# jameshball/kidney-diffusion

Measured on AMD Instinct MI355X. Metric: denoising-steps/sec (64->256 SR UNet, bs16), higher is better.
Workload: dtype f32

## Files before the change

### include/kd_engine.h

```cpp
#ifndef KD_ENGINE_H
#define KD_ENGINE_H

#include <stddef.h>
#include <stdint.h>

#ifdef __cplusplus
extern "C" {
#endif

#define KD_MAX_LEVELS 8

const char* kd_last_error(void);
#define KD_ENGINE_ABI_VERSION 2
int kd_version(void);
const char* kd_build_id(void);

typedef struct kd_unet_config {
  int dim;
  int num_levels;
  int dim_mults[KD_MAX_LEVELS];
  int num_resnet_blocks[KD_MAX_LEVELS];
  int layer_attns[KD_MAX_LEVELS];
  int layer_cross_attns[KD_MAX_LEVELS];
  int cond_dim;
// ... 184 lines not shown
                           float* d_part, int B, int H, int W, int heads, void* stream);
int kd_linattn_context(const float* d_k, const float* d_v, int ld, const float* d_part, int HW, const float* d_ck,
                       const float* d_cv, int ldc, int m, const float* d_null_k, const float* d_null_v, float* d_ctx, int B,
                       int heads, void* stream);
int kd_linattn_apply(const float* d_q, int ldq, const float* d_ctx, float* d_out, int ldo, int B, int N, int heads,
                     float scale, int silu, void* stream);
int kd_gn_fold_seg(const double* d_seg0, int nseg0, int nchunk0, float scale0, float ab_mul0, const double* d_seg1, int nseg1,
                   int nchunk1, float scale1, float ab_mul1, const float* d_gamma, const float* d_beta,
                   const float* d_scale_shift, int ld_ss, float* d_ab, float* d_stats, int B, int HW, int C, int G, float eps,
                   void* stream);
float kd_wf_ab_scale(void);
int kd_gn_conv3x3_winograd4_nhwc(const float* d_x, int ldx, const float* d_stats, const float* d_gamma, const float* d_beta,
                                 const float* d_scale_shift, int ld_ss, int skip_c0, float skip_scale, const float* d_w_oihw,
                                 const float* d_bias, const float* d_res, int ldres, float* d_y, double* d_out_seg, int B,
                                 int H, int W, int Cin, int Cout, int G, int gemm_mode, int images_per_set, void* stream);

int kd_init_conv_nchw(const float* d_x, const float* d_w3, const float* d_w7, const float* d_w15,
                      const float* d_bias, float* d_y, int B, int S, int n3, int n7, int n15, void* stream);
int kd_init_conv_planes_nchw(const float* d_x, const float* d_self_cond, const float* d_w3, const float* d_w7,
                             const float* d_w15, int Itot, int c0, const float* d_bias, const float* d_res, float* d_y, int B,
                             int S, int n3, int n7, int n15, int iters, float* ms, void* stream);
int kd_groupnorm_silu_nhwc(const float* d_x, const float* d_gamma, const float* d_beta,
                           const float* d_scale_shift, float* d_y, int B, int HW, int C, int G,
                           float eps, void* stream);
int kd_layernorm(const float* d_x, const float* d_g, const float* d_beta, float* d_y,
                 int rows, int C, float eps, void* stream);
int kd_layernorm_ex(const float* d_x, const float* d_g, const float* d_beta, const float* d_res, float* d_y, int rows, int C,
                    float eps, int in_act, const float* d_g2, float* d_y2, void* stream);
int kd_layernorm_linear_bf16x3(const float* d_x, const float* d_g, const float* d_beta, int rows, int C, float eps, int in_act,
                               const float* d_w, const float* d_bias, const float* d_res, int ldres, float* d_y, int ldy,
// ... 17 lines not shown
```

### kidney-diffusion_amd/csrc/api.inc

```
extern "C" {

const char* kd_last_error(void) { return kd::g_err.c_str(); }
int kd_version(void) { return KD_ENGINE_ABI_VERSION; }

int kd_unet_create(const kd_unet_config_t* cfg, const kd_param_t* params, int n_params, kd_unet_t** out) {
  return kd_unet_create_shared(cfg, params, n_params, nullptr, out);
}

int kd_unet_create_shared(const kd_unet_config_t* cfg, const kd_param_t* params, int n_params,
                          const kd_unet_t* share_with, kd_unet_t** out) {
  return kd_unet_create_self_cond(cfg, params, n_params, share_with, 0, out);
}

int kd_unet_create_self_cond(const kd_unet_config_t* cfg, const kd_param_t* params, int n_params,
                             const kd_unet_t* share_with, int self_cond, kd_unet_t** out) {
  kd_unet_ext_t ext;
  memset(&ext, 0, sizeof ext);
  ext.self_cond = self_cond;
  return kd_unet_create_ext(cfg, params, n_params, share_with, &ext, out);
}

int kd_unet_create_ext(const kd_unet_config_t* cfg, const kd_param_t* params, int n_params, const kd_unet_t* share_with,
                       const kd_unet_ext_t* ext, kd_unet_t** out) {
  const int self_cond = ext ? ext->self_cond : 0;
  if (!cfg || !params || !out) {
    set_error("kd_unet_create: null argument");
    return 1;
  }
  int ndev = 0;
  if (hipGetDeviceCount(&ndev) != hipSuccess || ndev == 0) {
    set_error("kd_unet_create: no HIP device visible — the engine has no CPU path");
    return 1;
  }
  if (share_with && (share_with->self_cond != 0) != (self_cond != 0)) {
    set_error("kd_unet_create: a shared plan must have the same self_cond");
    return 1;
  }
  kd_unet* u = new kd_unet();
  u->cfg = *cfg;
  u->self_cond = self_cond != 0;
  if (ext)
    for (int l = 0; l < KD_MAX_LEVELS; ++l) {
      u->lin_attn[l] = l < cfg->num_levels && ext->use_linear_attn[l] != 0;
      u->lin_cross[l] = l < cfg->num_levels && ext->use_linear_cross_attn[l] != 0;
    }
  u->wstore = share_with ? share_with->wstore : std::make_shared<WeightStore>();
  try {
    Builder b(u);
    for (int i = 0; i < n_params; ++i) {
      if (!params[i].name || !params[i].d_data) throw std::runtime_error("parameter table has a null entry");
      b.params[params[i].name] = {params[i].d_data, params[i].numel};
    }
    b.build();
    u->ws_bytes = b.arena.peak;
// ... 563 lines not shown
                 16 * (nseg0 + (d_seg1 ? nseg1 : 0)) == C,
             "kd_gn_fold_seg: the sources' 16-channel segments must tile the C channels");
  KD_REQUIRE(!d_ab || (d_gamma && d_beta), "kd_gn_fold_seg: the affine needs gamma and beta");
  KD_REQUIRE(!d_scale_shift || ld_ss >= 2 * C, "kd_gn_fold_seg: FiLM rows [scale | shift] need ld_ss >= 2 C");
  SegSrc s0{d_seg0, nseg0, nchunk0, 0, scale0, ab_mul0};
  SegSrc s1{d_seg1, d_seg1 ? nseg1 : 0, d_seg1 ? nchunk1 : 0, 16 * nseg0, scale1, ab_mul1};
  return entry_finish(launch_gn_fold_seg(s0, s1, d_gamma, d_beta, d_scale_shift, ld_ss, d_ab, d_stats, B, C, G,
                                         (double)HW * (C / G), eps, s),
                      s);
}

int kd_gn_conv3x3_winograd4_nhwc(const float* d_x, int ldx, const float* d_stats, const float* d_gamma, const float* d_beta,
                                 const float* d_scale_shift, int ld_ss, int skip_c0, float skip_scale, const float* d_w_oihw,
                                 const float* d_bias, const float* d_res, int ldres, float* d_y, double* d_out_seg, int B,
                                 int H, int W, int Cin, int Cout, int G, int gemm_mode, int images_per_set, void* stream) {
  hipStream_t s = (hipStream_t)stream;
  if (ldx <= 0) ldx = Cin;
  if (ldres <= 0) ldres = Cout;
  const int Bx = images_per_set > 0 ? images_per_set : B;
  KD_REQUIRE(d_x && d_stats && d_gamma && d_beta && d_w_oihw && d_bias && d_y, "kd_gn_conv3x3_winograd4_nhwc: null argument");
  KD_REQUIRE(B > 0 && Bx > 0 && B % Bx == 0, "kd_gn_conv3x3_winograd4_nhwc: images_per_set must divide B");
  KD_REQUIRE(H > 0 && W > 0 && H % 4 == 0 && W % 4 == 0, "Winograd F(4x4,3x3) path needs H % 4 == 0 and W % 4 == 0");
  const int64_t Mt = (int64_t)Bx * (H / 4) * (W / 4);
  KD_REQUIRE(Mt % 128 == 0 && Cin % 32 == 0 && Cout % 64 == 0 && 36 * Mt < 0x7fffffff &&
                 (int64_t)36 * Cout * Cin * 4 < 0x7fffffff,
             "Winograd F(4x4,3x3) path needs images_per_set*H*W/16 % 128 == 0, Cin % 32 == 0, Cout % 64 == 0");
  KD_REQUIRE(gemm_mode == -1 || gemm_mode == 1 || gemm_mode == 2, "kd_gn_conv3x3_winograd4_nhwc: gemm_mode -1, 1 or 2");
  KD_REQUIRE(gemm_mode < 0 || gemm_bf16x3_ok(36, Mt, Cout, Cin),
             "bf16x3 position GEMMs need images_per_set*H*W/16 % 256 == 0, Cout % 128 == 0, Cin % 32 == 0");
  KD_REQUIRE(G > 0 && Cin % G == 0, "kd_gn_conv3x3_winograd4_nhwc: Cin % G == 0");
// ... 4 lines not shown
  KD_REQUIRE(!d_res || (ldres >= Cout && ldres % 2 == 0), "kd_gn_conv3x3_winograd4_nhwc: residual row stride >= Cout, even");
  KD_REQUIRE((((uintptr_t)d_y | (uintptr_t)d_res | (uintptr_t)d_bias) & 7) == 0,
             "kd_gn_conv3x3_winograd4_nhwc: 8-byte aligned y, residual and bias");
  const bool planes = gemm_mode == 1, x3 = gemm_mode > 0;
  EntryBufs bufs;
  float *U = nullptr, *D = nullptr;
  void *V = nullptr, *U3 = nullptr, *ws = nullptr;
  if (bufs.get((void**)&U, (size_t)36 * Cout * Cin * sizeof(float))) return 1;
  if (bufs.get(&V, planes ? (size_t)36 * Mt * Cin * 6 : (size_t)36 * Mt * Cin * sizeof(float))) return 1;
  if (bufs.get((void**)&D, (size_t)36 * Mt * Cout * sizeof(float))) return 1;
  if (x3 && bufs.get(&U3, ((size_t)36 * Cout * Cin * 3 + 1) / 2 * sizeof(float))) return 1;
  if (x3 && bufs.get(&ws, gemm_bf16x3_workspace_bytes())) return 1;
  int rc = launch_wino4_pack(d_w_oihw, U, Cout, Cin, s);
  if (!rc && x3) rc = launch_split3(U, U3, 36, Cout, Cin, s);
  const int64_t HW = (int64_t)H * W, nchunk = (H / 4) * (W / 4);
  for (int st = 0; st < B / Bx && !rc; ++st) {
    const int b0 = st * Bx;
    const float* xs = d_x + (size_t)b0 * HW * ldx;
    const float* ss = d_stats + (size_t)b0 * G * 2;
    const float* ssp = d_scale_shift ? d_scale_shift + (size_t)b0 * ld_ss : nullptr;
    if (planes)
      rc = launch_wino4_in3(xs, ldx, ss, d_gamma, d_beta, ssp, ld_ss, V, Bx, H, W, Cin, G, s, skip_c0, skip_scale);
    else
      rc = launch_wino4_in(xs, ldx, ss, d_gamma, d_beta, ssp, ld_ss, (float*)V, Bx, H, W, Cin, G, s, skip_c0, skip_scale);
    if (!rc && x3) {
      rc = launch_gemm_bf16x3(V, U3, D, 36, (int)Mt, Cout, Cin, ws, s, !planes, false);
      if (!rc && gemm_bf16x3_needs_sum(36, (int)Mt, Cout, Cin)) rc = launch_gemm_bf16x3_sum(D, 36, (int)Mt, Cout, Cin, ws, s);
    } else if (!rc) {
      ConvParams p{};
      p.x = (const float*)V; p.w = U; p.y = D;
      p.B = 1; p.Hi = 1; p.Wi = (int)(36 * Mt); p.Cin = Cin; p.ldx = Cin;
      p.Ho = 1; p.Wo = (int)(36 * Mt); p.Cout = Cout;
      p.KH = 1; p.KW = 1; p.stride = 1; p.pad = 0;
      p.out_mode = OUT_NHWC; p.ldy = Cout;
      p.wz_rows = (int)Mt; p.wz_count = 36;
      rc = launch_conv_igemm(p, s);
    }
    if (!rc)
      rc = launch_wino4_out(D, d_bias, d_res ? d_res + (size_t)b0 * HW * ldres : nullptr, ldres, d_y + (size_t)b0 * HW * Cout,
                            Cout, d_out_seg ? d_out_seg + (size_t)b0 * (Cout / 16) * nchunk * 2 : nullptr, Bx, H, W, Cout, s);
  }
  return entry_finish(rc, s);
}

int kd_init_conv_nchw(const float* d_x, const float* d_w3, const float* d_w7, const float* d_w15, const float* d_bias,
                      float* d_y, int B, int S, int n3, int n7, int n15, void* stream) {
  return kd_init_conv_planes_nchw(d_x, nullptr, d_w3, d_w7, d_w15, 3, 0, d_bias, nullptr, d_y, B, S, n3, n7, n15, 1, nullptr,
                                  stream);
}

int kd_init_conv_planes_nchw(const float* d_x, const float* d_self_cond, const float* d_w3, const float* d_w7,
                             const float* d_w15, int Itot, int c0, const float* d_bias, const float* d_res, float* d_y, int B,
                             int S, int n3, int n7, int n15, int iters, float* ms, void* stream) {
  hipStream_t s = (hipStream_t)stream;
  const int np = d_self_cond ? 6 : 3;
// ... 125 lines not shown
```

### kidney-diffusion_amd/csrc/common.h

```cpp
#pragma once
#include <hip/hip_runtime.h>
#include <stdint.h>
#include <stdio.h>
#include <algorithm>
#include <string>

#ifdef KD_EXPERIMENT
#include "../../scratch/experiment_switch.h"
#else
constexpr int kd_switch(const char*, int dflt) { return dflt; }
#endif

namespace kd {

void set_error(const std::string& msg);

#define KD_HIP_CHECK(expr)                                                               \
  do {                                                                                   \
    hipError_t _e = (expr);                                                              \
    if (_e != hipSuccess) {                                                              \
      ::kd::set_error(std::string(#expr) + " failed: " + hipGetErrorString(_e) + " at " + \
                      __FILE__ + ":" + std::to_string(__LINE__));                        \
      return 1;                                                                          \
    }                                                                                    \
// ... 49 lines not shown
int launch_pack_unshuffle(const float* w, float* w_packed, int O, int C, hipStream_t s);
int launch_pack_shuffle(const float* w, const float* b, float* w_packed, float* b_packed, int Co, int I,
                        hipStream_t s);

int launch_wino_pack(const float* w_oihw, float* U, int O, int I, hipStream_t s);
int launch_wino_in(const float* x, int ldx, const float* stats, const float* gamma, const float* beta,
                   const float* scale_shift, int ld_ss, float* V, int B, int H, int W, int C, int G, int64_t t0,
                   int64_t nt, hipStream_t s);
int launch_wino_out(const float* D, const float* bias, const float* res, int ldres, float* y, int B, int H, int W,
                    int C, int64_t t0, int64_t nt, hipStream_t s, double* seg_partial = nullptr);

int launch_wino4_pack(const float* w_oihw, float* U, int O, int I, hipStream_t s);
int launch_wino4_in(const float* x, int ldx, const float* stats, const float* gamma, const float* beta,
                    const float* scale_shift, int ld_ss, float* V, int B, int H, int W, int C, int G, hipStream_t s,
                    int mul_c0 = -1, float mul = 1.0f);
int launch_wino4_out(const float* D, const float* bias, const float* res, int ldres, float* y, int ldy, double* seg_partial,
                     int B, int H, int W, int C, hipStream_t s);

constexpr int X3_BK = 16;
__device__ __forceinline__ void x3_split(const float __attribute__((ext_vector_type(2))) a, uint32_t& h, uint32_t& m,
                                         uint32_t& l) {
  typedef float f2 __attribute__((ext_vector_type(2)));
  typedef __bf16 b2 __attribute__((ext_vector_type(2)));
  const b2 hb = __builtin_convertvector(a, b2);
  const f2 r1 = a - __builtin_convertvector(hb, f2);
  const b2 mb = __builtin_convertvector(r1, b2);
  const f2 r2 = r1 - __builtin_convertvector(mb, f2);
  const b2 lb = __builtin_convertvector(r2, b2);
  h = __builtin_bit_cast(uint32_t, hb);
  m = __builtin_bit_cast(uint32_t, mb);
  l = __builtin_bit_cast(uint32_t, lb);
}
bool gemm_bf16x3_ok(int G, int64_t M, int N, int K);
int launch_split3(const float* x, void* planes, int G, int R, int K, hipStream_t s);
// ... 10 lines not shown
  int a_tap_c = 0, a_wi = 0, a_hi = 0;
  double* seg = nullptr;
  int seg_nseg = 0, seg_coff = 0;
  int seg_rows8 = 0;
  int wide = 0;
  int act = ACT_NONE;
  int pixshuf_wo = 0;
};
bool gemm_bf16x3_epi_ok(int64_t M, int N, int K, const X3Epi& e);
int launch_gemm_bf16x3(const void* A3, const void* B3, float* C, int G, int M, int N, int K, void* ws, hipStream_t s,
                       bool a_f32 = false, bool with_sum = true, const X3Epi* epi = nullptr);
bool gemm_bf16x3_needs_sum(int G, int M, int N, int K);
int gemm_bf16x3_seg_rows(int M, int N, int K);
int launch_gemm_bf16x3_sum(float* C, int G, int M, int N, int K, const void* ws, hipStream_t s, const X3Epi* epi = nullptr);
int gemm_bf16x3_workgroups(int G, int M, int N, int K);
int launch_wino4_in3(const float* x, int ldx, const float* stats, const float* gamma, const float* beta,
                     const float* scale_shift, int ld_ss, void* V3, int B, int H, int W, int C, int G, hipStream_t s,
                     int mul_c0 = -1, float mul = 1.0f);

constexpr float WF_AB_SCALE = -1.4426950408889634f;
constexpr float WF_U_SCALE = -0.6931471805599453f;
int launch_gn_fold(const float* stats, const float* gamma, const float* beta, const float* scale_shift, int ld_ss,
                   float* ab, int B, int C, int G, hipStream_t s);
bool wino_fused128_ok(int B, int H, int W, int C, int N);
int launch_wino_fused128_pack(const float* w_oihw, float* U, int O, int I, hipStream_t s, float scale);
size_t wino_fused128_items_count(int B, int H, int W, int N);
int launch_wino_fused128_items(void* items, int B, int H, int W, int N, hipStream_t s);
size_t wino_fused_out_stats_chunks(int H, int W, int N, int G);
int launch_wino_fused_gn128(const float* x, int ldx, const float* ab, const float* U, const float* bias, const float* res,
                            int ldres, float* y, int B, int H, int W, int C, int N, double* out_partial, int out_groups,
// ... 140 lines not shown
```

### kidney-diffusion_amd/csrc/engine.hip

```cpp
#include <stdlib.h>
#include <string.h>

#include <algorithm>
#include <functional>
#include <map>
#include <memory>
#include <stdexcept>
#include <string>
#include <unordered_map>
#include <unordered_set>
#include <vector>

#include "../../include/kd_engine.h"
#include "common.h"

namespace kd {

static thread_local std::string g_err;
void set_error(const std::string& msg) { g_err = msg; }

#define KD_THROW_IF(expr)                                          \
  do {                                                             \
    if ((expr) != 0) throw std::runtime_error(::kd::g_err);        \
  } while (0)
// ... 194 lines not shown
  void drop_graphs() {
    ddpm_graph.drop();
    for (auto& g : edm_graph) g.drop();
  }
  ~Sampler() {
    if (cap_stream) (void)hipStreamDestroy(cap_stream);
  }
};

}

using namespace kd;

struct kd_unet {
  kd_unet_config_t cfg;
  std::vector<std::function<int(hipStream_t)>> ops;
  std::vector<std::string> op_label;
  std::vector<int64_t> op_macs;
  std::vector<int64_t> op_mfma;
  std::shared_ptr<WeightStore> wstore;
  char* ws = nullptr;
  size_t ws_bytes = 0;
  int64_t macs = 0;
  int64_t mfma_macs = 0;
  int64_t mfma_bf16_macs = 0;
  int time_cond_dim = 0;
  int self_cond = 0;
  int lin_attn[KD_MAX_LEVELS] = {0};
  int lin_cross[KD_MAX_LEVELS] = {0};
  const float *in_x = nullptr, *in_lowres = nullptr, *in_cond = nullptr, *in_log_snr = nullptr,
// ... 816 lines not shown
  }
  T wino4_block(const T& x, int Bx, const std::string& gn_prefix, int ss_col, const std::string& conv_prefix, int Cout,
                const T* res, int skip_c0, float skip_scale) {
    const int Cin = x.C, G = cfg.resnet_groups, H = x.H, W = x.W, HW = x.HW(), nset = x.B / Bx;
    const int64_t Mt = (int64_t)Bx * (H / 4) * (W / 4);
    const float* gamma = P(gn_prefix + ".weight", Cin);
    const float* beta = P(gn_prefix + ".bias", Cin);
    const float* bias = P(conv_prefix + ".bias", Cout);
    const float* wsrc = raw(conv_prefix + ".weight", (int64_t)Cout * Cin * 9);
    float* U = cached("wino4:" + conv_prefix, (size_t)36 * Cout * Cin,
                      [&](float* dst) { KD_THROW_IF(launch_wino4_pack(wsrc, dst, Cout, Cin, 0)); });
    emit_gn_stats(x, gamma, beta, ss_col, nullptr);
    const bool x3 = cfg.gemm_bf16x3 >= 0 && !to_text && !to_static && gemm_bf16x3_ok(36, Mt, Cout, Cin);
    const bool v_f32 = cfg.gemm_bf16x3 == 2 || (cfg.gemm_bf16x3 == 0 && (int64_t)Cin * Cout < 40 * (6 * (int64_t)Cin + 4 * Cout));
    const bool x3_planes = x3 && !v_f32;
    T V = x3_planes ? alloc_bytes((size_t)36 * Mt * Cin * 6) : alloc(1, 1, (int)(36 * Mt), Cin);
    T D = alloc(1, 1, (int)(36 * Mt), Cout);
    T y = alloc(x.B, H, W, Cout);
    const std::string shape = " M" + std::to_string((int64_t)Bx * HW) + " Cin" + std::to_string(Cin) + " Cout" +
                              std::to_string(Cout);
    kd_unet* uu = u;
    const bool sg = Cout % 64 == 0;
    const size_t sgo_all = sg ? add_seg(y, 0, Cout / 16, (H / 4) * (W / 4)) : 0;
    for (int st = 0; st < nset; ++st) {
      const int b0 = st * Bx;
      {
        size_t xo = x.at() + (size_t)b0 * HW * x.LD() * sizeof(float), vo = V.off;
        size_t so = gn_stats_t.off + (size_t)b0 * G * 2 * sizeof(float), sso = t_ss.off + (size_t)b0 * tmlp_total * sizeof(float);
        const int ld = tmlp_total, ldx = x.LD();
        emit([=](hipStream_t s) {
// ... 2 lines not shown
            return launch_wino4_in3(uu->P(xo), ldx, uu->P(so), gamma, beta, ssp, ld, uu->P(vo), Bx, H, W, Cin, G, s, skip_c0, skip_scale);
          return launch_wino4_in(uu->P(xo), ldx, uu->P(so), gamma, beta, ssp, ld, uu->P(vo), Bx, H, W, Cin, G, s, skip_c0, skip_scale);
        }, (x3_planes ? "wino4_in3" : "wino4_in") + shape);
      }
      if (x3) {
        const float* U3 = cached("wino4x3:" + conv_prefix, ((size_t)36 * Cout * Cin * 3 + 1) / 2,
                                 [&](float* dst) { KD_THROW_IF(launch_split3(U, dst, 36, Cout, Cin, 0)); });
        const size_t vo = V.off, d_o = D.off;
        const int64_t macs = (int64_t)Bx * HW * Cout * Cin * 9;
        if (!u->x3_ws) KD_HIP_THROW(hipMalloc(&u->x3_ws, gemm_bf16x3_workspace_bytes()));
        emit([=](hipStream_t s) { return launch_gemm_bf16x3(uu->P(vo), U3, uu->P(d_o), 36, (int)Mt, Cout, Cin, uu->x3_ws, s, !x3_planes, false); },
             "wino4 gemm bf16x3" + shape, macs);
        u->macs += macs;
        u->op_mfma.back() = 6 * 36 * Mt * Cout * Cin;
        u->mfma_bf16_macs += u->op_mfma.back();
        if (gemm_bf16x3_needs_sum(36, (int)Mt, Cout, Cin))
          emit([=](hipStream_t s) { return launch_gemm_bf16x3_sum(uu->P(d_o), 36, (int)Mt, Cout, Cin, uu->x3_ws, s); },
               "wino4 x3 sum" + shape);
      } else {
        ConvOpt o;
        o.wz_rows = (int)Mt;
        o.wz_count = 36;
        o.dst = &D;
        o.macs_override = (int64_t)Bx * HW * Cout * Cin * 9;
        conv(V, U, nullptr, Cout, 1, 1, 0, o);
        if (!to_text && !to_static) u->op_label.back() = "wino4 gemm" + shape;
      }
      {
        const size_t sgo = sgo_all + (size_t)b0 * (Cout / 16) * ((H / 4) * (W / 4)) * 2 * sizeof(double);
        size_t d_o = D.off, yo = y.off + (size_t)b0 * HW * Cout * sizeof(float);
        const bool hr = res != nullptr;
        const int ldres = res ? res->LD() : 0;
        size_t ro = res ? res->at() + (size_t)b0 * HW * ldres * sizeof(float) : 0;
        emit([=](hipStream_t s) {
          return launch_wino4_out(uu->P(d_o), bias, hr ? uu->P(ro) : nullptr, ldres, uu->P(yo), Cout,
                                  sg ? (double*)uu->P(sgo) : nullptr, Bx, H, W, Cout, s);
        }, "wino4_out" + shape);
      }
    }
    free(V);
    free(D);
    return y;
  }

  T wino_block(const T& x, const std::string& gn_prefix, int ss_col, const std::string& conv_prefix, int Cout,
               const T* res) {
    const int Cin = x.C, G = cfg.resnet_groups, Bx = x.B, H = x.H, W = x.W, HW = x.HW();
    const int64_t Mt = (int64_t)Bx * (H / 2) * (W / 2);
    const float* gamma = P(gn_prefix + ".weight", Cin);
    const float* beta = P(gn_prefix + ".bias", Cin);
    const float* bias = P(conv_prefix + ".bias", Cout);
// ... 403 lines not shown
```

### kidney-diffusion_amd/csrc/kernels_gemm_bf16x3.hip

```cpp
#include "common.h"
#include "epilogue.h"

namespace kd {

namespace {

typedef float f32x16 __attribute__((ext_vector_type(16)));
typedef float f32x2 __attribute__((ext_vector_type(2)));
typedef short bf16x8 __attribute__((ext_vector_type(8)));
typedef __bf16 bf16x2 __attribute__((ext_vector_type(2)));
typedef int i32x4 __attribute__((ext_vector_type(4)));

constexpr int BM = 256, BN = 128, BK = X3_BK;
constexpr int ROWB = BK * 2;
constexpr int NST = 4;
constexpr int STAGE_B = 3 * (BM + BN) * ROWB;
constexpr int B_OFF = 3 * BM * ROWB;

__device__ __forceinline__ void dma16(const i32x4& rsrc, uint32_t lds_addr, uint32_t voff, uint32_t soff) {
  asm volatile("s_mov_b32 m0, %0\n\ts_nop 0\n\tbuffer_load_dwordx4 %1, %2, %3 offen lds" ::"s"(lds_addr), "v"(voff), "s"(rsrc),
               "s"(soff)
               : "memory");
}
__device__ __forceinline__ i32x4 make_rsrc(const void* base, uint32_t bytes) {
  const uint64_t a = (uint64_t)(uintptr_t)base;
  i32x4 r;
  r[0] = __builtin_amdgcn_readfirstlane((int)(uint32_t)a);
  r[1] = __builtin_amdgcn_readfirstlane((int)(uint32_t)((a >> 32) & 0xffffu));
// ... 26 lines not shown
}

int launch_split3(const float* x, void* planes, int G, int R, int K, hipStream_t s) {
  KD_REQUIRE(K % BK == 0 && ((uintptr_t)x & 7) == 0, "bf16x3 planes need K % 16 == 0");
  const int64_t n2 = (int64_t)G * R * K / 2;
  hipLaunchKernelGGL(split3_kernel, dim3((unsigned)((n2 + 255) / 256)), dim3(256), 0, s, x, (uint32_t*)planes, n2, R, K);
  KD_HIP_CHECK(hipGetLastError());
  return 0;
}

template <int V>
struct X3Set { static constexpr int value = V; };
struct X3Yes { static constexpr bool value = true; };
struct X3No { static constexpr bool value = false; };
constexpr int X3_MAX_WG = 512;
constexpr int X3_MAX_SPLIT = 8;

template <bool A_F32, int EK>
__global__ __launch_bounds__(768) void gemm_bf16x3_kernel(const uint16_t* __restrict__ A3, const uint16_t* __restrict__ B3,
                                                          float* __restrict__ C, int G, int M, int N, int K, int S_st,
                                                          float* __restrict__ slab, X3Epi e) {
  constexpr bool EPI = EK != 0;
  const int S = S_st & 0xff, stagger = S_st >> 8;
  const int lda = EPI ? e.lda : K, ldc = EPI ? e.ldy : N;
  constexpr int EPI_LDS = EK == 1 ? 8 * 2048 : 0;
  __shared__ __attribute__((aligned(1024))) char lds[NST * STAGE_B + EPI_LDS];
  const int tid = threadIdx.x, lane = tid & 63;
  const int wave = __builtin_amdgcn_readfirstlane(tid >> 6);
  const int mtiles = M / BM, ntiles = N / BN;
  const int nk = K / BK;
  const int P = gridDim.x;
// ... 582 lines not shown
int gemm_bf16x3_workgroups(int G, int M, int N, int K) {
  int P, R, S, first;
  x3_shape(G, M, N, K, &P, &R, &S, &first);
  return P;
}
size_t gemm_bf16x3_workspace_bytes() {
  return (size_t)X3_MAX_WG * BM * BN * sizeof(float);
}

int gemm_bf16x3_seg_rows(int M, int N, int K) { return gemm_bf16x3_needs_sum(1, M, N, K) ? 8 : 32; }
bool gemm_bf16x3_needs_sum(int G, int M, int N, int K) {
  int P, R, S, first;
  x3_shape(G, M, N, K, &P, &R, &S, &first);
  return R && S > 1;
}
int launch_gemm_bf16x3_sum(float* C, int G, int M, int N, int K, const void* ws, hipStream_t s, const X3Epi* epi) {
  int P, R, S, first;
  x3_shape(G, M, N, K, &P, &R, &S, &first);
  if (!(R && S > 1)) return 0;
  if (epi)
    hipLaunchKernelGGL(sum_slabs_kernel<true>, dim3((unsigned)(R * 32)), dim3(256), 0, s, (const float*)ws, C, G, M, N, S, first, *epi);
  else
    hipLaunchKernelGGL(sum_slabs_kernel<false>, dim3((unsigned)(R * 32)), dim3(256), 0, s, (const float*)ws, C, G, M, N, S, first,
                       X3Epi{});
  KD_HIP_CHECK(hipGetLastError());
  return 0;
}

bool gemm_bf16x3_epi_ok(int64_t M, int N, int K, const X3Epi& e) {
  if (!gemm_bf16x3_ok(1, M, N, K)) return false;
// ... 57 lines not shown
```

### kidney-diffusion_amd/csrc/kernels_wino4.hip

```cpp
#include "common.h"

namespace kd {

namespace {
__device__ __forceinline__ float w4_silu(float v) {
  return v * __builtin_amdgcn_rcpf(1.0f + __builtin_amdgcn_exp2f(-1.4426950408889634f * v));
}

typedef float f32x2 __attribute__((ext_vector_type(2)));

template <class F>
__device__ __forceinline__ void w4_bt(const F (&d)[6], F (&t)[6]) {
  t[0] = 4.0f * d[0] - 5.0f * d[2] + d[4];
  t[1] = (d[3] + d[4]) - 4.0f * (d[1] + d[2]);
  t[2] = (d[4] - d[3]) + 4.0f * (d[1] - d[2]);
  t[3] = (d[4] - d[2]) + 2.0f * (d[3] - d[1]);
  t[4] = (d[4] - d[2]) + 2.0f * (d[1] - d[3]);
  t[5] = 4.0f * d[1] - 5.0f * d[3] + d[5];
}
template <class F>
__device__ __forceinline__ void w4_at(const F (&m)[6], F (&y)[4]) {
  const F a = m[1] + m[2], b = m[1] - m[2], c = m[3] + m[4], d = m[3] - m[4];
  y[0] = m[0] + a + c;
  y[1] = b + 2.0f * d;
// ... 174 lines not shown
                     const float* scale_shift, int ld_ss, void* V3, int B, int H, int W, int C, int G, hipStream_t s, int mul_c0,
                     float mul) {
  KD_REQUIRE(mul_c0 < 0 || stats, "Winograd F(4x4,3x3) input transform: a channel scale needs the GroupNorm form");
  if (mul_c0 < 0) mul_c0 = C;
  const int64_t nt = (int64_t)B * (H / 4) * (W / 4), total = nt * (C / 2);
  KD_REQUIRE((int64_t)B * H * W * ldx * 4 < ((int64_t)1 << 32), "Winograd F(4x4,3x3) input transform: maps below 4 GB");
  KD_REQUIRE(H % 4 == 0 && W % 4 == 0 && ldx >= C && C % X3_BK == 0 && ldx % 2 == 0 && ((uintptr_t)x & 7) == 0 && nt % 8 == 0 &&
                 ((uintptr_t)V3 & 3) == 0,
             "Winograd F(4x4,3x3) input transform to bf16x3 planes needs H % 4 == 0, W % 4 == 0, C % 16 == 0, tiles % 8 == 0");
  hipLaunchKernelGGL(wino4_in_kernel<true>, dim3((unsigned)((total + 255) / 256)), dim3(256), 0, s, x, ldx, stats, gamma, beta,
                     scale_shift, ld_ss, (float*)V3, B, H, W, C, G, nt, mul_c0, mul);
  KD_HIP_CHECK(hipGetLastError());
  return 0;
}

template <bool RES>
__global__ __launch_bounds__(256) void wino4_out_kernel(const float* __restrict__ D, const float* __restrict__ bias,
                                                        const float* __restrict__ res, int ldres, float* __restrict__ y,
                                                        int ldy, double* __restrict__ seg, int B, int H, int W, int C,
                                                        int64_t nt) {
  const int Ht = H >> 2, Wt = W >> 2, C2 = C >> 1;
  const int64_t idx = (int64_t)blockIdx.x * blockDim.x + threadIdx.x;
  if (idx >= nt * C2) return;
  const int c = (int)(idx % C2) * 2;
  const int64_t t = idx / C2;
  const int tx = (int)(t % Wt);
  const int ty = (int)((t / Wt) % Ht);
  const int b = (int)(t / ((int64_t)Wt * Ht));
  const float* in = D + t * C + c;
  const int64_t pstride = nt * C;
  f32x2 u[4][6];
#pragma unroll
  for (int s = 0; s < 6; ++s) {
    f32x2 m[6];
#pragma unroll
    for (int r = 0; r < 6; ++r) m[r] = *(const f32x2*)(in + (int64_t)(r * 6 + s) * pstride);
    f32x2 ycol[4];
    w4_at(m, ycol);
#pragma unroll
    for (int i = 0; i < 4; ++i) u[i][s] = ycol[i];
  }
  f32x2 bv = {0.0f, 0.0f};
  if (bias) bv = *(const f32x2*)(bias + c);
  f32x2 rnext[4];
#pragma unroll
  for (int j = 0; j < 4; ++j) rnext[j] = f32x2{0.0f, 0.0f};
  const int64_t pix0 = ((int64_t)b * H + 4 * ty) * W + 4 * tx;
  if (RES) {
#pragma unroll
    for (int j = 0; j < 4; ++j) rnext[j] = *(const f32x2*)(res + (pix0 + j) * ldres + c);
  }
  float s1 = 0.0f, s2 = 0.0f;
#pragma unroll
// ... 22 lines not shown
#pragma unroll
    for (int off = 1; off <= 4; off <<= 1) {
      d1 += __shfl_xor(d1, off, 64);
      d2 += __shfl_xor(d2, off, 64);
    }
    if ((c & 15) == 0) {
      const int nchunk = Ht * Wt;
      double* op = seg + (((int64_t)b * (C >> 4) + (c >> 4)) * nchunk + (ty * Wt + tx)) * 2;
      op[0] = d1;
      op[1] = d2;
    }
  }
}

int launch_wino4_out(const float* D, const float* bias, const float* res, int ldres, float* y, int ldy, double* seg_partial,
                     int B, int H, int W, int C, hipStream_t s) {
  KD_REQUIRE(H % 4 == 0 && W % 4 == 0 && ldy >= C && C % 2 == 0 && ldy % 2 == 0 && ldres % 2 == 0 &&
                 (((uintptr_t)y | (uintptr_t)res | (uintptr_t)bias) & 7) == 0,
             "Winograd F(4x4,3x3) output transform needs H % 4 == 0, W % 4 == 0, even C / row strides, 8-byte aligned maps");
  KD_REQUIRE(!seg_partial || C % 128 == 0 || (C % 16 == 0 && ((int64_t)B * (H / 4) * (W / 4) * (C / 2)) % 64 == 0),
             "output statistics need whole waves of 16-channel segments");
  const int64_t nt = (int64_t)B * (H / 4) * (W / 4), total = nt * (C / 2);
  if (res)
    hipLaunchKernelGGL(wino4_out_kernel<true>, dim3((unsigned)((total + 255) / 256)), dim3(256), 0, s, D, bias, res, ldres, y, ldy,
                       seg_partial, B, H, W, C, nt);
  else
    hipLaunchKernelGGL(wino4_out_kernel<false>, dim3((unsigned)((total + 255) / 256)), dim3(256), 0, s, D, bias, res, ldres, y, ldy,
                       seg_partial, B, H, W, C, nt);
  KD_HIP_CHECK(hipGetLastError());
  return 0;
}

}
```

### kidney-diffusion_amd/imagen_pytorch/_engine.py

```python
from __future__ import annotations

import ctypes as C
import os
from pathlib import Path

KD_MAX_LEVELS = 8

_LIB_PATH = Path(__file__).resolve().parent.parent / "lib" / "libkd_engine.so"


class EngineUnavailable(RuntimeError):
    pass


class EngineError(RuntimeError):
    pass


class kd_unet_config_t(C.Structure):
    _fields_ = [
        ("dim", C.c_int),
        ("num_levels", C.c_int),
        ("dim_mults", C.c_int * KD_MAX_LEVELS),
        ("num_resnet_blocks", C.c_int * KD_MAX_LEVELS),
# ... 136 lines not shown
    "kd_linattn_context": (C.c_int, [C.c_void_p, C.c_void_p, C.c_int, C.c_void_p, C.c_int, C.c_void_p, C.c_void_p, C.c_int,
                                     C.c_int, C.c_void_p, C.c_void_p, C.c_void_p, C.c_int, C.c_int, C.c_void_p]),
    "kd_linattn_apply": (C.c_int, [C.c_void_p, C.c_int, C.c_void_p, C.c_void_p, C.c_int, C.c_int, C.c_int, C.c_int,
                                   C.c_float, C.c_int, C.c_void_p]),
    "kd_linear_skinny": (C.c_int, [C.c_void_p, C.c_int, C.c_void_p, C.c_void_p, C.c_void_p] + [C.c_int] * 6 + [C.c_void_p]),
    "kd_global_context_gate": (C.c_int, [C.c_void_p] + [C.c_int] * 3 + [C.c_void_p] * 4 + [C.c_int] + [C.c_void_p] * 4 +
                               [C.c_int, C.c_void_p]),
    "kd_gate_add_nhwc": (C.c_int, [C.c_void_p] * 3 + [C.c_int, C.c_void_p, C.c_int, C.c_void_p] + [C.c_int] * 3 + [C.c_void_p]),
    "kd_gate_add_chunks": (C.c_int, [C.c_int, C.c_int]),
    "kd_gn_fold_seg": (C.c_int, [C.c_void_p, C.c_int, C.c_int, C.c_float, C.c_float, C.c_void_p, C.c_int, C.c_int, C.c_float,
                                 C.c_float] + [C.c_void_p] * 3 + [C.c_int] + [C.c_void_p] * 2 + [C.c_int] * 4 +
                       [C.c_float, C.c_void_p]),
    "kd_wf_ab_scale": (C.c_float, []),
    "kd_gn_conv3x3_winograd4_nhwc": (C.c_int, [C.c_void_p, C.c_int] + [C.c_void_p] * 4 + [C.c_int, C.c_int, C.c_float] +
                                     [C.c_void_p] * 3 + [C.c_int] + [C.c_void_p] * 2 + [C.c_int] * 8 + [C.c_void_p]),
    "kd_init_conv_nchw": (C.c_int, [C.c_void_p] * 6 + [C.c_int] * 5 + [C.c_void_p]),
    "kd_init_conv_planes_nchw": (C.c_int, [C.c_void_p] * 5 + [C.c_int] * 2 + [C.c_void_p] * 3 + [C.c_int] * 6 +
                                 [C.POINTER(C.c_float), C.c_void_p]),
    "kd_groupnorm_silu_nhwc": (C.c_int, [C.c_void_p] * 5 + [C.c_int] * 4 + [C.c_float, C.c_void_p]),
    "kd_layernorm": (C.c_int, [C.c_void_p] * 4 + [C.c_int, C.c_int, C.c_float, C.c_void_p]),
    "kd_layernorm_ex": (C.c_int, [C.c_void_p] * 5 + [C.c_int, C.c_int, C.c_float, C.c_int, C.c_void_p, C.c_void_p, C.c_void_p]),
    "kd_layernorm_linear_bf16x3": (C.c_int, [C.c_void_p] * 3 + [C.c_int, C.c_int, C.c_float, C.c_int] + [C.c_void_p] * 3 +
                                   [C.c_int, C.c_void_p, C.c_int, C.c_int, C.c_void_p, C.c_void_p]),
    "kd_attention": (C.c_int, [C.c_void_p] * 4 + [C.c_int] * 6 + [C.c_void_p]),
    "kd_attention_ex": (C.c_int, [C.c_void_p, C.c_int, C.c_void_p, C.c_void_p, C.c_void_p, C.c_int, C.c_int, C.c_void_p,
                                  C.c_void_p, C.c_int, C.c_int, C.c_void_p, C.c_int, C.c_int, C.c_int, C.c_int, C.c_int,
                                  C.c_float, C.c_void_p]),
    "kd_l2norm_heads": (C.c_int, [C.c_void_p, C.c_int, C.c_int64, C.c_int, C.c_void_p, C.c_void_p]),
    "kd_quantile_abs": (C.c_int, [C.c_void_p, C.c_void_p, C.c_int, C.c_int64, C.c_float, C.c_void_p, C.c_size_t,
                                  C.c_void_p]),
# ... 90 lines not shown
```

Measured before the change: 40.61.

## Fuse split-K slab reduction into Winograd output transform

When the bf16x3 GEMM splits K across slabs, the Winograd output transform now reads and sums the per-split partial slabs itself instead of running a separate sum kernel that writes D first. This removes one kernel launch and one full write-and-read round trip of D per Winograd conv. In exchange the output kernel issues more scattered buffer loads using a swizzled slab layout, and it carries more register pressure from holding the full 6x6 tile. A config flag (gemm_bf16x3 >= 4) restores the old separate sum launch.

```diff
diff --git a/include/kd_engine.h b/include/kd_engine.h
--- a/include/kd_engine.h
+++ b/include/kd_engine.h
@@ -222,6 +222,12 @@
                                  const float* d_scale_shift, int ld_ss, int skip_c0, float skip_scale, const float* d_w_oihw,
                                  const float* d_bias, const float* d_res, int ldres, float* d_y, double* d_out_seg, int B,
                                  int H, int W, int Cin, int Cout, int G, int gemm_mode, int images_per_set, void* stream);
+int kd_gn_conv3x3_winograd4_sums_nhwc(const float* d_x, int ldx, const float* d_stats, const float* d_gamma, const float* d_beta,
+                                      const float* d_scale_shift, int ld_ss, int skip_c0, float skip_scale, const float* d_w_oihw,
+                                      const float* d_bias, const float* d_res, int ldres, float* d_y, double* d_out_seg, int B,
+                                      int H, int W, int Cin, int Cout, int G, int gemm_mode, int images_per_set, int out_sums,
+                                      void* stream);
+int kd_gemm_bf16x3_split(int G, int M, int N, int K);
 
 int kd_init_conv_nchw(const float* d_x, const float* d_w3, const float* d_w7, const float* d_w15,
                       const float* d_bias, float* d_y, int B, int S, int n3, int n7, int n15, void* stream);
diff --git a/kidney-diffusion_amd/csrc/api.inc b/kidney-diffusion_amd/csrc/api.inc
--- a/kidney-diffusion_amd/csrc/api.inc
+++ b/kidney-diffusion_amd/csrc/api.inc
@@ -38,6 +38,10 @@
   }
   kd_unet* u = new kd_unet();
   u->cfg = *cfg;
+  if (u->cfg.gemm_bf16x3 >= 4) {
+    u->x3_sum_launch = true;
+    u->cfg.gemm_bf16x3 -= 4;
+  }
   u->self_cond = self_cond != 0;
   if (ext)
     for (int l = 0; l < KD_MAX_LEVELS; ++l) {
@@ -631,6 +635,20 @@
                                  const float* d_scale_shift, int ld_ss, int skip_c0, float skip_scale, const float* d_w_oihw,
                                  const float* d_bias, const float* d_res, int ldres, float* d_y, double* d_out_seg, int B,
                                  int H, int W, int Cin, int Cout, int G, int gemm_mode, int images_per_set, void* stream) {
+  return kd_gn_conv3x3_winograd4_sums_nhwc(d_x, ldx, d_stats, d_gamma, d_beta, d_scale_shift, ld_ss, skip_c0, skip_scale, d_w_oihw,
+                                           d_bias, d_res, ldres, d_y, d_out_seg, B, H, W, Cin, Cout, G, gemm_mode, images_per_set, 0,
+                                           stream);
+}
+
+int kd_gemm_bf16x3_split(int G, int M, int N, int K) {
+  return G > 0 && M > 0 && N > 0 && K > 0 && gemm_bf16x3_ok(G, M, N, K) ? gemm_bf16x3_slabs(G, M, N, K, nullptr).S : 0;
+}
+
+int kd_gn_conv3x3_winograd4_sums_nhwc(const float* d_x, int ldx, const float* d_stats, const float* d_gamma, const float* d_beta,
+                                      const float* d_scale_shift, int ld_ss, int skip_c0, float skip_scale, const float* d_w_oihw,
+                                      const float* d_bias, const float* d_res, int ldres, float* d_y, double* d_out_seg, int B,
+                                      int H, int W, int Cin, int Cout, int G, int gemm_mode, int images_per_set, int out_sums,
+                                      void* stream) {
   hipStream_t s = (hipStream_t)stream;
   if (ldx <= 0) ldx = Cin;
   if (ldres <= 0) ldres = Cout;
@@ -665,6 +683,7 @@
   int rc = launch_wino4_pack(d_w_oihw, U, Cout, Cin, s);
   if (!rc && x3) rc = launch_split3(U, U3, 36, Cout, Cin, s);
   const int64_t HW = (int64_t)H * W, nchunk = (H / 4) * (W / 4);
+  X3Slabs slabs;
   for (int st = 0; st < B / Bx && !rc; ++st) {
     const int b0 = st * Bx;
     const float* xs = d_x + (size_t)b0 * HW * ldx;
@@ -676,7 +695,8 @@
       rc = launch_wino4_in(xs, ldx, ss, d_gamma, d_beta, ssp, ld_ss, (float*)V, Bx, H, W, Cin, G, s, skip_c0, skip_scale);
     if (!rc && x3) {
       rc = launch_gemm_bf16x3(V, U3, D, 36, (int)Mt, Cout, Cin, ws, s, !planes, false);
-      if (!rc && gemm_bf16x3_needs_sum(36, (int)Mt, Cout, Cin)) rc = launch_gemm_bf16x3_sum(D, 36, (int)Mt, Cout, Cin, ws, s);
+      if (out_sums >= 0) slabs = gemm_bf16x3_slabs(36, (int)Mt, Cout, Cin, ws);
+      else if (!rc && gemm_bf16x3_needs_sum(36, (int)Mt, Cout, Cin)) rc = launch_gemm_bf16x3_sum(D, 36, (int)Mt, Cout, Cin, ws, s);
     } else if (!rc) {
       ConvParams p{};
       p.x = (const float*)V; p.w = U; p.y = D;
@@ -689,7 +709,7 @@
     }
     if (!rc)
       rc = launch_wino4_out(D, d_bias, d_res ? d_res + (size_t)b0 * HW * ldres : nullptr, ldres, d_y + (size_t)b0 * HW * Cout,
-                            Cout, d_out_seg ? d_out_seg + (size_t)b0 * (Cout / 16) * nchunk * 2 : nullptr, Bx, H, W, Cout, s);
+                            Cout, d_out_seg ? d_out_seg + (size_t)b0 * (Cout / 16) * nchunk * 2 : nullptr, Bx, H, W, Cout, s, &slabs);
   }
   return entry_finish(rc, s);
 }
diff --git a/kidney-diffusion_amd/csrc/common.h b/kidney-diffusion_amd/csrc/common.h
--- a/kidney-diffusion_amd/csrc/common.h
+++ b/kidney-diffusion_amd/csrc/common.h
@@ -87,10 +87,13 @@
 int launch_wino4_in(const float* x, int ldx, const float* stats, const float* gamma, const float* beta,
                     const float* scale_shift, int ld_ss, float* V, int B, int H, int W, int C, int G, hipStream_t s,
                     int mul_c0 = -1, float mul = 1.0f);
+struct X3Slabs;
 int launch_wino4_out(const float* D, const float* bias, const float* res, int ldres, float* y, int ldy, double* seg_partial,
-                     int B, int H, int W, int C, hipStream_t s);
+                     int B, int H, int W, int C, hipStream_t s, const X3Slabs* slabs = nullptr);
 
 constexpr int X3_BK = 16;
+constexpr int X3_BM = 256, X3_BN = 128;
+constexpr int X3_MAX_SPLIT = 8;
 __device__ __forceinline__ void x3_split(const float __attribute__((ext_vector_type(2))) a, uint32_t& h, uint32_t& m,
                                          uint32_t& l) {
   typedef float f2 __attribute__((ext_vector_type(2)));
@@ -131,6 +134,12 @@
 int gemm_bf16x3_seg_rows(int M, int N, int K);
 int launch_gemm_bf16x3_sum(float* C, int G, int M, int N, int K, const void* ws, hipStream_t s, const X3Epi* epi = nullptr);
 int gemm_bf16x3_workgroups(int G, int M, int N, int K);
+struct X3Slabs {
+  const float* slab = nullptr;
+  uint32_t bytes = 0;
+  int S = 0, first_tile = 0;
+};
+X3Slabs gemm_bf16x3_slabs(int G, int M, int N, int K, const void* ws);
 int launch_wino4_in3(const float* x, int ldx, const float* stats, const float* gamma, const float* beta,
                      const float* scale_shift, int ld_ss, void* V3, int B, int H, int W, int C, int G, hipStream_t s,
                      int mul_c0 = -1, float mul = 1.0f);
diff --git a/kidney-diffusion_amd/csrc/engine.hip b/kidney-diffusion_amd/csrc/engine.hip
--- a/kidney-diffusion_amd/csrc/engine.hip
+++ b/kidney-diffusion_amd/csrc/engine.hip
@@ -232,6 +232,7 @@
 
 struct kd_unet {
   kd_unet_config_t cfg;
+  bool x3_sum_launch = false;
   std::vector<std::function<int(hipStream_t)>> ops;
   std::vector<std::string> op_label;
   std::vector<int64_t> op_macs;
@@ -1078,6 +1079,7 @@
     const bool x3 = cfg.gemm_bf16x3 >= 0 && !to_text && !to_static && gemm_bf16x3_ok(36, Mt, Cout, Cin);
     const bool v_f32 = cfg.gemm_bf16x3 == 2 || (cfg.gemm_bf16x3 == 0 && (int64_t)Cin * Cout < 40 * (6 * (int64_t)Cin + 4 * Cout));
     const bool x3_planes = x3 && !v_f32;
+    const bool out_sums = x3 && !u->x3_sum_launch;
     T V = x3_planes ? alloc_bytes((size_t)36 * Mt * Cin * 6) : alloc(1, 1, (int)(36 * Mt), Cin);
     T D = alloc(1, 1, (int)(36 * Mt), Cout);
     T y = alloc(x.B, H, W, Cout);
@@ -1110,7 +1112,7 @@
         u->macs += macs;
         u->op_mfma.back() = 6 * 36 * Mt * Cout * Cin;
         u->mfma_bf16_macs += u->op_mfma.back();
-        if (gemm_bf16x3_needs_sum(36, (int)Mt, Cout, Cin))
+        if (gemm_bf16x3_needs_sum(36, (int)Mt, Cout, Cin) && !out_sums)
           emit([=](hipStream_t s) { return launch_gemm_bf16x3_sum(uu->P(d_o), 36, (int)Mt, Cout, Cin, uu->x3_ws, s); },
                "wino4 x3 sum" + shape);
       } else {
@@ -1129,8 +1131,9 @@
         const int ldres = res ? res->LD() : 0;
         size_t ro = res ? res->at() + (size_t)b0 * HW * ldres * sizeof(float) : 0;
         emit([=](hipStream_t s) {
+          const X3Slabs sl = out_sums ? gemm_bf16x3_slabs(36, (int)Mt, Cout, Cin, uu->x3_ws) : X3Slabs{};
           return launch_wino4_out(uu->P(d_o), bias, hr ? uu->P(ro) : nullptr, ldres, uu->P(yo), Cout,
-                                  sg ? (double*)uu->P(sgo) : nullptr, Bx, H, W, Cout, s);
+                                  sg ? (double*)uu->P(sgo) : nullptr, Bx, H, W, Cout, s, &sl);
         }, "wino4_out" + shape);
       }
     }
diff --git a/kidney-diffusion_amd/csrc/kernels_gemm_bf16x3.hip b/kidney-diffusion_amd/csrc/kernels_gemm_bf16x3.hip
--- a/kidney-diffusion_amd/csrc/kernels_gemm_bf16x3.hip
+++ b/kidney-diffusion_amd/csrc/kernels_gemm_bf16x3.hip
@@ -11,7 +11,7 @@
 typedef __bf16 bf16x2 __attribute__((ext_vector_type(2)));
 typedef int i32x4 __attribute__((ext_vector_type(4)));
 
-constexpr int BM = 256, BN = 128, BK = X3_BK;
+constexpr int BM = X3_BM, BN = X3_BN, BK = X3_BK;
 constexpr int ROWB = BK * 2;
 constexpr int NST = 4;
 constexpr int STAGE_B = 3 * (BM + BN) * ROWB;
@@ -68,7 +68,6 @@
 struct X3Yes { static constexpr bool value = true; };
 struct X3No { static constexpr bool value = false; };
 constexpr int X3_MAX_WG = 512;
-constexpr int X3_MAX_SPLIT = 8;
 
 template <bool A_F32, int EK>
 __global__ __launch_bounds__(768) void gemm_bf16x3_kernel(const uint16_t* __restrict__ A3, const uint16_t* __restrict__ B3,
@@ -681,6 +680,17 @@
   x3_shape(G, M, N, K, &P, &R, &S, &first);
   return R && S > 1;
 }
+X3Slabs gemm_bf16x3_slabs(int G, int M, int N, int K, const void* ws) {
+  int P, R, S, first;
+  x3_shape(G, M, N, K, &P, &R, &S, &first);
+  X3Slabs sl;
+  if (!(R && S > 1)) return sl;
+  sl.slab = (const float*)ws;
+  sl.bytes = (uint32_t)((size_t)R * S * BM * BN * sizeof(float));
+  sl.S = S;
+  sl.first_tile = first;
+  return sl;
+}
 int launch_gemm_bf16x3_sum(float* C, int G, int M, int N, int K, const void* ws, hipStream_t s, const X3Epi* epi) {
   int P, R, S, first;
   x3_shape(G, M, N, K, &P, &R, &S, &first);
diff --git a/kidney-diffusion_amd/csrc/kernels_wino4.hip b/kidney-diffusion_amd/csrc/kernels_wino4.hip
--- a/kidney-diffusion_amd/csrc/kernels_wino4.hip
+++ b/kidney-diffusion_amd/csrc/kernels_wino4.hip
@@ -212,11 +212,11 @@
   return 0;
 }
 
-template <bool RES>
+template <bool RES, bool SLAB>
 __global__ __launch_bounds__(256) void wino4_out_kernel(const float* __restrict__ D, const float* __restrict__ bias,
                                                         const float* __restrict__ res, int ldres, float* __restrict__ y,
                                                         int ldy, double* __restrict__ seg, int B, int H, int W, int C,
-                                                        int64_t nt) {
+                                                        int64_t nt, X3Slabs sl) {
   const int Ht = H >> 2, Wt = W >> 2, C2 = C >> 1;
   const int64_t idx = (int64_t)blockIdx.x * blockDim.x + threadIdx.x;
   if (idx >= nt * C2) return;
@@ -227,14 +227,63 @@
   const int b = (int)(t / ((int64_t)Wt * Ht));
   const float* in = D + t * C + c;
   const int64_t pstride = nt * C;
+  int tpp = 0, lt0 = -(1 << 24);
+  if (SLAB) {
+    const int ntiles = C / X3_BN;
+    tpp = (int)(nt / X3_BM) * ntiles;
+    lt0 = __builtin_amdgcn_readfirstlane((int)(t / X3_BM) * ntiles + c / X3_BN) - sl.first_tile;
+  }
+  f32x2 m[6][6];
+  if (SLAB) {
+    const int row = (int)(t % X3_BM), col = c % X3_BN;
+    const uint32_t voff = (uint32_t)((((((row >> 5) & 1) * 2 + ((col >> 5) & 1)) * 4 + ((row >> 3) & 3)) * 512 +
+                                      ((row >> 6) * 2 + (col >> 6)) * 64 + ((row >> 2) & 1) * 32 + (col & 31)) * 16 + (row & 3) * 4);
+    const __amdgpu_buffer_rsrc_t rsS = __builtin_amdgcn_make_buffer_rsrc((void*)sl.slab, 0, (int)sl.bytes, 0x00020000);
+    constexpr uint32_t SLAB_B = X3_BM * X3_BN * 4;
+    __builtin_assume(sl.S >= 2 && sl.S <= X3_MAX_SPLIT);
+#pragma unroll
+    for (int r = 0; r < 6; ++r)
+#pragma unroll
+      for (int s = 0; s < 6; ++s) {
+        const int lt = (r * 6 + s) * tpp + lt0;
+        if (lt < 0) continue;
+        constexpr int NQ = 6;
+        static_assert(X3_MAX_SPLIT == NQ + 2, "the parts of a position: six, then two");
+        auto load_part = [&](int q) __attribute__((always_inline)) {
+          const uint32_t so = (uint32_t)(lt * sl.S + (q < sl.S ? q : sl.S - 1)) * SLAB_B;
+          return f32x2{__uint_as_float(__builtin_amdgcn_raw_buffer_load_b32(rsS, voff, so, 0)),
+                       __uint_as_float(__builtin_amdgcn_raw_buffer_load_b32(rsS, voff, so + 16, 0))};
+        };
+        f32x2 part[NQ];
+#pragma unroll
+        for (int q = 0; q < NQ; ++q) part[q] = load_part(q);
+        f32x2 v = part[0];
+#pragma unroll
+        for (int q = 1; q < NQ; ++q) v = q < sl.S ? v + part[q] : v;
+        if (sl.S > NQ) {
+          const f32x2 p6 = load_part(NQ), p7 = load_part(NQ + 1);
+          v = v + p6;
+          v = NQ + 1 < sl.S ? v + p7 : v;
+        }
+        m[r][s] = v;
+      }
+  }
+#pragma unroll
+  for (int r = 0; r < 6; ++r)
+#pragma unroll
+    for (int s = 0; s < 6; ++s) {
+      const int p = r * 6 + s;
+      if (SLAB && p * tpp + lt0 >= 0) continue;
+      m[r][s] = *(const f32x2*)(in + (int64_t)p * pstride);
+    }
   f32x2 u[4][6];
 #pragma unroll
   for (int s = 0; s < 6; ++s) {
-    f32x2 m[6];
-#pragma unroll
-    for (int r = 0; r < 6; ++r) m[r] = *(const f32x2*)(in + (int64_t)(r * 6 + s) * pstride);
+    f32x2 mc[6];
+#pragma unroll
+    for (int r = 0; r < 6; ++r) mc[r] = m[r][s];
     f32x2 ycol[4];
-    w4_at(m, ycol);
+    w4_at(mc, ycol);
 #pragma unroll
     for (int i = 0; i < 4; ++i) u[i][s] = ycol[i];
   }
@@ -287,19 +336,26 @@
 }
 
 int launch_wino4_out(const float* D, const float* bias, const float* res, int ldres, float* y, int ldy, double* seg_partial,
-                     int B, int H, int W, int C, hipStream_t s) {
+                     int B, int H, int W, int C, hipStream_t s, const X3Slabs* slabs) {
   KD_REQUIRE(H % 4 == 0 && W % 4 == 0 && ldy >= C && C % 2 == 0 && ldy % 2 == 0 && ldres % 2 == 0 &&
                  (((uintptr_t)y | (uintptr_t)res | (uintptr_t)bias) & 7) == 0,
              "Winograd F(4x4,3x3) output transform needs H % 4 == 0, W % 4 == 0, even C / row strides, 8-byte aligned maps");
   KD_REQUIRE(!seg_partial || C % 128 == 0 || (C % 16 == 0 && ((int64_t)B * (H / 4) * (W / 4) * (C / 2)) % 64 == 0),
              "output statistics need whole waves of 16-channel segments");
   const int64_t nt = (int64_t)B * (H / 4) * (W / 4), total = nt * (C / 2);
-  if (res)
-    hipLaunchKernelGGL(wino4_out_kernel<true>, dim3((unsigned)((total + 255) / 256)), dim3(256), 0, s, D, bias, res, ldres, y, ldy,
-                       seg_partial, B, H, W, C, nt);
-  else
-    hipLaunchKernelGGL(wino4_out_kernel<false>, dim3((unsigned)((total + 255) / 256)), dim3(256), 0, s, D, bias, res, ldres, y, ldy,
-                       seg_partial, B, H, W, C, nt);
+  const bool slab = slabs && slabs->S > 1;
+  KD_REQUIRE(!slab || (slabs->slab && C % X3_BN == 0 && nt % X3_BM == 0 && slabs->S <= X3_MAX_SPLIT && slabs->first_tile >= 0 &&
+                       36 * (nt / X3_BM) * (C / X3_BN) < (1 << 24) && ((uintptr_t)slabs->slab & 3) == 0),
+             "Winograd F(4x4,3x3) output transform over k-part slabs needs C % 128 == 0, tiles % 256 == 0 and at most 8 parts");
+  const dim3 grid((unsigned)((total + 255) / 256)), block(256);
+  const X3Slabs sl = slab ? *slabs : X3Slabs{};
+#define KD_W4OUT(R, S) hipLaunchKernelGGL((wino4_out_kernel<R, S>), grid, block, 0, s, D, bias, res, ldres, y, ldy, seg_partial, B, H, W, C, nt, sl)
+  if (res) {
+    if (slab) KD_W4OUT(true, true); else KD_W4OUT(true, false);
+  } else {
+    if (slab) KD_W4OUT(false, true); else KD_W4OUT(false, false);
+  }
+#undef KD_W4OUT
   KD_HIP_CHECK(hipGetLastError());
   return 0;
 }
diff --git a/kidney-diffusion_amd/imagen_pytorch/_engine.py b/kidney-diffusion_amd/imagen_pytorch/_engine.py
--- a/kidney-diffusion_amd/imagen_pytorch/_engine.py
+++ b/kidney-diffusion_amd/imagen_pytorch/_engine.py
@@ -174,6 +174,9 @@
     "kd_wf_ab_scale": (C.c_float, []),
     "kd_gn_conv3x3_winograd4_nhwc": (C.c_int, [C.c_void_p, C.c_int] + [C.c_void_p] * 4 + [C.c_int, C.c_int, C.c_float] +
                                      [C.c_void_p] * 3 + [C.c_int] + [C.c_void_p] * 2 + [C.c_int] * 8 + [C.c_void_p]),
+    "kd_gn_conv3x3_winograd4_sums_nhwc": (C.c_int, [C.c_void_p, C.c_int] + [C.c_void_p] * 4 + [C.c_int, C.c_int, C.c_float] +
+                                          [C.c_void_p] * 3 + [C.c_int] + [C.c_void_p] * 2 + [C.c_int] * 9 + [C.c_void_p]),
+    "kd_gemm_bf16x3_split": (C.c_int, [C.c_int] * 4),
     "kd_init_conv_nchw": (C.c_int, [C.c_void_p] * 6 + [C.c_int] * 5 + [C.c_void_p]),
     "kd_init_conv_planes_nchw": (C.c_int, [C.c_void_p] * 5 + [C.c_int] * 2 + [C.c_void_p] * 3 + [C.c_int] * 6 +
                                  [C.POINTER(C.c_float), C.c_void_p]),
```

New measurement: 39.70. 2.2% lower.
